# Gaurav14cs17/Bayer_Low_light_Image_Enhancement

Measured on AMD Instinct MI355X. Metric: megapixels/sec RawFormer-S 512x512 RAW->sRGB, higher is better.
Workload: dtype f32; 1 GPU; RawFormer-S(FLCA) dim=32, batch=8 of packed 4x512x512 synthetic Bayer per GPU; frames_per_gpu=8, variant=flca, weights=synthetic (seeded, random-init scale), parallelism=batch-sharded x1, device=AMD Radeon Graphics

## Files before the change

bayer_low_light_image_enhancement_amd/csrc/rf_block.hip:

```cpp
#include <cstdlib>
#include "rf_common.h"

namespace rf {

size_t transformer_scratch_floats(int B, int C, int heads, int hc, int h, int w, TbBufOffsets* o) {
    const size_t P = (size_t)h * w;
    Bump b;
    const size_t wide = (size_t)(3 * C > hc ? 3 * C : hc);
    o->bufA = b.off((size_t)B * wide * P);
    o->bufB = b.off((size_t)B * wide * P);
    o->x1 = b.off((size_t)B * C * P);
    int ns, sl;
    size_t pf = 0, pf2 = 0;
    if (gram_plan(B, C, heads, (int)P, &ns, &sl, &pf)) return 0;
    if (fused_attn_supported(C, heads, h, w)) fused_attn_plan(h, w, &ns, &pf2, B, C);
    if (attn_mid_supported(C, heads, h, w)) attn_mid_plan(h, w, &ns, &pf2, B, C);
    o->partial = b.off(pf > pf2 ? pf : pf2);
    o->wfold = b.off((size_t)B * packed1x1_floats(C, C));
    o->wfold3 = b.off((size_t)B * packed1x1_b3_floats(C, C));
    return b.used;
}

bool transformer_ffn_is_fused(const TbParams& p, int C, int hc, int hh, int ww) {
#ifdef RF_DIAG
// ... 31 lines not shown
            RF_TRY(launch_attn_mid(buf.pre, buf.qkv, partial, nslab, p.qkv_dw_w, p.qkv_dw_b, B, C, hh, ww, st, p.ylo, p.yhi, p.xlo, p.xhi));
            av.x1 = buf.qkv; av.x1_bstride = (int64_t)C * Pn;
        } else {
            DwConvArgs d{};
            d.x = buf.pre; d.x_bstride = (int64_t)3 * C * Pn; d.out = buf.qkv; d.out_bstride = (int64_t)3 * C * Pn;
            d.w = p.qkv_dw_w; d.bias = p.qkv_dw_b;
            d.B = B; d.C = 3 * C; d.h = hh; d.w_ = ww; d.gelu = 0;
            RF_TRY(launch_dwconv3x3(d, st));

            GramArgs g{};
            g.q = buf.qkv; g.k = buf.qkv + (size_t)C * Pn; g.bstride = (int64_t)3 * C * Pn;
            g.B = B; g.C = C; g.heads = heads; g.P = Pn; g.partial = partial;
            RF_TRY(gram_plan(B, C, heads, Pn, &g.nslab, &g.slab, &partial_floats));
            g.p_lo = p.ylo * ww; g.p_hi = p.yhi * ww;
            if (p.xhi > 0 && (p.xlo > 0 || p.xhi < ww)) { g.w = ww; g.x_lo = p.xlo; g.x_hi = p.xhi; }
            RF_TRY(launch_gram(g, st));
            nslab = g.nslab;
            av.x1 = buf.qkv + (size_t)2 * C * Pn; av.x1_bstride = (int64_t)3 * C * Pn;
        }
    }
    if (p.allreduce) p.allreduce(p.allreduce_user, partial, partial_floats, 0, (void*)st);
    RF_TRY(launch_attn_fold(partial, nslab, p.temperature, p.proj_w, buf.wfold, buf.wfold3, B, C, heads, st, p.log_temperature));
    av.C1 = C;
    av.wp = buf.wfold; av.wp_bstride = (int64_t)packed1x1_floats(C, C);
    av.wp3 = buf.wfold3; av.wp3_bstride = (int64_t)packed1x1_b3_floats(C, C);
    av.bias = p.proj_b;
    if (residual) { av.res = in; av.res_bstride = (int64_t)C * Pn; }
    av.out = out; av.out_bstride = (int64_t)C * Pn; av.Cout = C; av.B = B; av.P = Pn; av.w = ww;
    return launch_conv1x1(av, st);
}

int run_transformer(const TbParams& p, const float* in, float* out, float* ws, const TbBufOffsets& o,
                    int B, int C, int heads, int hc, int hh, int ww, hipStream_t st) {
    const int Pn = hh * ww;
    float* bufA = ws + o.bufA;
    float* bufB = ws + o.bufB;
    float* x1 = ws + o.x1;
#ifdef RF_DIAG
    const bool no_fuse = getenv("RF_NO_FUSE") != nullptr;
    const bool no_fuse_attn = no_fuse || getenv("RF_NO_FUSE_ATTN") != nullptr;
#else
    constexpr bool no_fuse = false, no_fuse_attn = false;
#endif

    RF_TRY(run_chan_attn(p, in, x1, true, AttnBufs{bufA, bufB, ws + o.partial, ws + o.wfold, ws + o.wfold3}, B, C, heads, hh, ww, st, no_fuse,
                         no_fuse_attn));

    if (transformer_ffn_is_fused(p, C, hc, hh, ww)) {
        RF_TRY(launch_ffn_fused(x1, out, p.ln2_w, p.ln2_b, p.pw1_wp3, p.pw1_b, p.dw_w, p.dw_b, p.pw2_wp, p.pw2_b, B, C, hh, ww, st));
    } else {
        Conv1x1Args f1{};
        f1.x1 = x1; f1.C1 = C; f1.x1_bstride = (int64_t)C * Pn;
        f1.wp = p.pw1_wp; f1.wp3 = p.pw1_wp3; f1.bias = p.pw1_b;
        f1.ln_w = p.ln2_w; f1.ln_b = p.ln2_b; f1.ln_eps = 1e-5f;
        f1.out = bufA; f1.out_bstride = (int64_t)hc * Pn; f1.Cout = hc; f1.B = B; f1.P = Pn; f1.w = ww;
        if (!conv1x1_ln_single_pass(f1)) {
            RF_TRY(launch_layernorm2d(x1, bufB, p.ln2_w, p.ln2_b, 1e-5f, B, C, Pn, st));
            f1.x1 = bufB; f1.ln_w = nullptr; f1.ln_b = nullptr;
        }
        RF_TRY(launch_conv1x1(f1, st));

        DwConvArgs d2{};
        d2.x = bufA; d2.x_bstride = (int64_t)hc * Pn; d2.out = bufB; d2.out_bstride = (int64_t)hc * Pn;
        d2.w = p.dw_w; d2.bias = p.dw_b;
        d2.B = B; d2.C = hc; d2.h = hh; d2.w_ = ww; d2.gelu = 1;
        RF_TRY(launch_dwconv3x3(d2, st));
        if (p.defer_pw2) return RF_OK;

        Conv1x1Args f2{};
        f2.x1 = bufB; f2.C1 = hc; f2.x1_bstride = (int64_t)hc * Pn;
        f2.wp = p.pw2_wp; f2.wp3 = p.pw2_wp3; f2.bias = p.pw2_b;
        f2.res = x1; f2.res_bstride = (int64_t)C * Pn;
        f2.out = out; f2.out_bstride = (int64_t)C * Pn; f2.Cout = C; f2.B = B; f2.P = Pn; f2.w = ww;
        RF_TRY(launch_conv1x1(f2, st));
    }
    return RF_OK;
}

}
```

bayer_low_light_image_enhancement_amd/csrc/rf_common.h:

```cpp
#pragma once
#include <hip/hip_runtime.h>
#include <stdint.h>
#include <stddef.h>
#include "../../include/rawformer_hip.h"

namespace rf {

typedef float f32x4 __attribute__((ext_vector_type(4)));

void set_error(const char* fmt, ...);
int check_hip(hipError_t e, const char* what);
int check_launch(const char* what);

#define RF_CHECK_ARG(cond, ...)            \
    do {                                   \
        if (!(cond)) {                     \
            rf::set_error(__VA_ARGS__);    \
            return RF_E_INVALID;           \
        }                                  \
    } while (0)

#define RF_TRY(expr)            \
    do {                        \
        const int rc_ = (expr); \
// ... 168 lines not shown
struct DwConvArgs {
    const float* x; int64_t x_bstride;
    float* out; int64_t out_bstride;
    const float* w;
    const float* bias;
    int B, C, h, w_;
    int gelu;
    float* out2 = nullptr;
};
int launch_dwconv3x3(const DwConvArgs& a, hipStream_t st);
int launch_pixel_unshuffle2(const float* in, float* out, int B, int C, int h, int w, hipStream_t st);
int launch_pixel_shuffle2(const float* in, float* out, int B, int C, int h, int w, hipStream_t st);
int launch_dwt2x2(const float* in, float* out, const float k[16], int layout, int exact_haar,
                  int B, int C, int h, int w, int hin, int win, hipStream_t st);
int launch_idwt2x2(const float* in, float* out, const float k[16], int layout, int exact_haar,
                   int B, int C, int h, int w, hipStream_t st);

struct GramArgs {
    const float* q; const float* k;
    int64_t bstride;
    int B, C, heads, P;
    float* partial;
    int nslab, slab;
    int p_lo = 0, p_hi = 0;
    int w = 0, x_lo = 0, x_hi = 0;
};
int gram_plan(int B, int C, int heads, int P, int* nslab, int* slab, size_t* partial_floats);
int launch_gram(const GramArgs& a, hipStream_t st);
int launch_attn_fold(const float* partial, int nslab, const float* temperature, const float* w_out,
                     float* wp_out, void* wp3_out , int B, int C, int heads, hipStream_t st,
                     int log_temperature = 0);

bool fused_ffn_supported(int C, int hidden, int h, int w);
int launch_ffn_fused(const float* x, float* out, const float* ln_w, const float* ln_b, const void* w1p , const float* b1,
                     const float* wd, const float* bd, const float* w2p, const float* b2, int B, int C, int h, int w, hipStream_t st);
bool fused_attn_supported(int C, int heads, int h, int w);
int fused_attn_plan(int h, int w, int* nslab, size_t* partial_floats, int B, int C);
int launch_attn_front(const float* x, float* v, float* partial, int nslab, const float* ln_w, const float* ln_b,
                      const void* wp , const float* bq, const float* wd, const float* bd, int B, int C, int h, int w, hipStream_t st,
                      int ylo = 0, int yhi = 0 ,
                      int xlo = 0, int xhi = 0 );

bool attn_mid_supported(int C, int heads, int h, int w);
int attn_mid_plan(int h, int w, int* nslab, size_t* partial_floats, int B, int C);
int launch_attn_mid(const float* qkv, float* v, float* partial, int nslab, const float* wd, const float* bd,
                    int B, int C, int h, int w, hipStream_t st, int ylo = 0, int yhi = 0, int xlo = 0, int xhi = 0);

struct TbParams {
    const float *ln1_w, *ln1_b, *temperature;
    const float *qkv_wp , *qkv_b, *qkv_dw_w, *qkv_dw_b, *proj_w , *proj_b;
    const float *ln2_w, *ln2_b, *pw1_wp , *pw1_b, *dw_w, *dw_b, *pw2_wp , *pw2_b;
    const void *qkv_wp3, *pw1_wp3, *pw2_wp3;
    int log_temperature;
    int ylo = 0, yhi = 0, xlo = 0, xhi = 0;
    void (*allreduce)(void* user, float* buf, size_t n, int op, void* stream) = nullptr;
    void* allreduce_user = nullptr;
    bool defer_pw2 = false;
};
bool transformer_ffn_is_fused(const TbParams& p, int C, int hc, int hh, int ww);
struct TbBufOffsets { size_t bufA, bufB, x1, partial, wfold, wfold3; };
size_t transformer_scratch_floats(int B, int C, int heads, int hc, int h, int w, TbBufOffsets* o);
int run_transformer(const TbParams& p, const float* in, float* out, float* ws, const TbBufOffsets& o,
                    int B, int C, int heads, int hc, int hh, int ww, hipStream_t st);
struct AttnBufs {
    float *pre, *qkv;
    float *partial;
    float *wfold;
    void* wfold3;
};
int run_chan_attn(const TbParams& p, const float* in, float* out, bool residual, const AttnBufs& buf, int B, int C, int heads, int hh, int ww,
                  hipStream_t st, bool no_fuse = false, bool no_fuse_attn = false);

int launch_rfft2_polar(const float* in, float* mag, float* pha, float2* cscratch, int planes, int h, int w, hipStream_t st);
int launch_polar_irfft2(const float* mag, const float* pha, const float* res, float* out, float2* cscratch, int planes, int h, int w,
                        float lim, hipStream_t st);
int launch_clamp(const float* in, float* out, size_t n, float lo, float hi, hipStream_t st);

size_t tc_front_scratch_floats(int B, int H, int W, int levels);
int launch_tc_front(const float* in, int mosaic, const float* wb_gains, const float* color_matrix, const float* wp_c0, const float* b_c0,
                    const float* wp_c2, const float* b_c2, const float* wp_d0, const float* b_d0, const float* wp_d2, const float* b_d2,
                    float* scratch, int B, int H, int W, int levels, hipStream_t st);
int launch_tc_guide_level(const float* scratch, float* guide, int B, int H, int W, int levels, int hf, int wf, hipStream_t st);
int tc_front_outputs(const float* scratch, const float** y, const float** crcb, const float** rgb, int B, int H, int W, int levels);
int tc_nblk(int h, int w);
int launch_tc_spatial(const float* feat, float* xs, const float* guide, const float* w_col, const float* b_col, const float* w_low,
                      const float* b_low, const float* w_high, const float* b_high, int B, int C, int h, int w, hipStream_t st);
int launch_tc_residual(const float* xs, const float* r, float* x2, float* partial, int B, int C, int h, int w, hipStream_t st);
int launch_tc_color_head(float* x, const float* const* prm, int B, size_t P, hipStream_t st);

size_t gram2_partial_floats(int B, int Ca, int Cb, int h, int w, int ntap);
struct Gram2Launch {
    const float* a; int64_t a_bstride; int Ca;
    const float* b; int64_t b_bstride; int Cb;
    const float* b2; int64_t b2_bstride; int Cb2;
    float* out; int ld;
    size_t out_istride;
// ... 73 lines not shown
```

bayer_low_light_image_enhancement_amd/csrc/rf_fused.hip:

```cpp
#include <cstdio>
#include <cstdlib>
#include "rf_common.h"

namespace rf {

#ifdef RF_STAMP
__device__ unsigned long long g_stamp[16];
#define STAMP_DECL unsigned long long st_prev = __builtin_amdgcn_s_memtime(), st_acc[8] = {0, 0, 0, 0, 0, 0, 0, 0};
#define STAMP(i) do { __builtin_amdgcn_sched_barrier(0); unsigned long long t_ = __builtin_amdgcn_s_memtime(); st_acc[i] += t_ - st_prev; st_prev = t_; __builtin_amdgcn_sched_barrier(0); } while (0)
#define STAMP_FLUSH do { if ((threadIdx.x & 63) == 0) for (int i_ = 0; i_ < 8; ++i_) atomicAdd(&g_stamp[i_], st_acc[i_]); } while (0)
#else
#define STAMP_DECL
#define STAMP(i)
#define STAMP_FLUSH
#endif

__device__ __forceinline__ void lds_barrier() {
    asm volatile("s_waitcnt lgkmcnt(0)" ::: "memory");
    __builtin_amdgcn_s_barrier();
    asm volatile("" ::: "memory");
}

namespace fused {
constexpr int TH = 4, TW = 64;
// ... 171 lines not shown
#pragma unroll
        for (int q = 0; q < 4; ++q) out[q] = fmaf(k2, v[q + 2], fmaf(k1, v[q + 1], fmaf(k0, v[q], out[q])));
    }
}

__device__ __forceinline__ void stencil4_wide(const float* __restrict__ p, const float* __restrict__ k9, float bias, float (&out)[4]) {
    using namespace fused;
#pragma unroll
    for (int q = 0; q < 4; ++q) out[q] = bias;
#pragma unroll
    for (int dy = 0; dy < 3; ++dy) {
        const float* row = p + dy * HC;
        const float4 lft = *reinterpret_cast<const float4*>(row - 4);
        const float4 m = *reinterpret_cast<const float4*>(row);
        const float4 rgt = *reinterpret_cast<const float4*>(row + 4);
        const float v[6] = {lft.w, m.x, m.y, m.z, m.w, rgt.x};
        const float k0 = k9[dy * 3], k1 = k9[dy * 3 + 1], k2 = k9[dy * 3 + 2];
#pragma unroll
        for (int q = 0; q < 4; ++q) out[q] = fmaf(k2, v[q + 2], fmaf(k1, v[q + 1], fmaf(k0, v[q], out[q])));
    }
}

struct FfnArgs {
    const float* x;
    float* out;
    const float* ln_w; const float* ln_b;
    const void* w1p;
    const float* b1;
    const float* wd;
    const float* bd;
    const float* w2p;
    const float* b2;
    int B, h, w, tiles_x, ntiles;
};

template <int C>
__global__ void __launch_bounds__(256, 2) ffn_fused_kernel(FfnArgs a) {
    using namespace fused;
    constexpr int NS = C / 4;
    constexpr int NT1 = 2 * C / 16;
    constexpr int NTO = C / 16;
    constexpr int NPART = 2 * C / PART;
    constexpr int PS = 448;
    __shared__ __attribute__((aligned(16))) float mid[PART * PS + 8];
    __shared__ __attribute__((aligned(16))) u32x4 w1_l[(C / 32) * NT1 * 192];
    __shared__ __attribute__((aligned(16))) float w2_l[(2 * C / 4) * NTO * 64];
    __shared__ float wd_l[2 * C * 9], bd_l[2 * C], b1_l[2 * C], b2_l[C], gam_l[C], bet_l[C];

    const int tid = threadIdx.x, lane = tid & 63, wave = tid >> 6;
    const int j = lane & 15, kq = lane >> 4;
    const int b = blockIdx.y;
    const int h = a.h, w = a.w, P = h * w;
    const float* xb = a.x + (size_t)b * C * P;
    float* ob = a.out + (size_t)b * C * P;

    for (int i = tid; i < (C / 32) * NT1 * 192; i += 256) w1_l[i] = reinterpret_cast<const u32x4*>(a.w1p)[i];
    for (int i = tid; i < (2 * C / 4) * NTO * 16; i += 256) *reinterpret_cast<float4*>(w2_l + i * 4) = *reinterpret_cast<const float4*>(a.w2p + i * 4);
    for (int i = tid; i < 2 * C * 9; i += 256) wd_l[i] = a.wd[i];
    for (int i = tid; i < 2 * C; i += 256) { bd_l[i] = a.bd[i]; b1_l[i] = a.b1[i]; }
    for (int i = tid; i < C; i += 256) { gam_l[i] = a.ln_w[i]; bet_l[i] = a.ln_b[i]; b2_l[i] = a.b2[i]; }
    __syncthreads();
    STAMP_DECL

    const int tiles_y = a.ntiles / a.tiles_x;
    const int per = (a.ntiles + (int)gridDim.x - 1) / (int)gridDim.x;
    const int t_begin = blockIdx.x * per, t_end = (t_begin + per < a.ntiles) ? t_begin + per : a.ntiles;
    for (int tile = t_begin; tile < t_end; ++tile) {
        const int tx = tile / tiles_y, ty = tile % tiles_y;
        const int x0 = tx * TW, y0 = ty * TH;
        STAMP(0);
        const GroupGeom gw0 = group_geom(wave, 0, j, y0, x0, h, w), gw1 = group_geom(wave, 1, j, y0, x0, h, w);
        u32x4 bp0[C / 32][4][3], bp1[C / 32][4][3];
        {
            float4 xh0[NS], xh1[NS];
            load_step_b3<C>(xb, P, kq, gw0, xh0);
            load_step_b3<C>(xb, P, kq, gw1, xh1);
            ln_step_b3<C>(kq, gam_l, bet_l, 1e-5f, xh0);
            ln_step_b3<C>(kq, gam_l, bet_l, 1e-5f, xh1);
            split_step<C>(xh0, bp0);
            split_step<C>(xh1, bp1);
        }
        STAMP(1);

        const int yo = y0 + wave, xo = x0 + 4 * j;
        const bool live = yo < h && xo < w;
        const unsigned voff = (unsigned)(4 * kq) * (unsigned)P + (unsigned)(live ? yo * w + xo : 0);
        float4 resv[NTO * 4];
        f32x4 acc[NTO][4];
#pragma unroll
        for (int t = 0; t < NTO; ++t)
#pragma unroll
            for (int q = 0; q < 4; ++q) acc[t][q] = (f32x4){0.f, 0.f, 0.f, 0.f};

#pragma unroll
        for (int part = 0; part < NPART; ++part) {
            lds_barrier();
            STAMP(0);
            phase_a_step_b3<C, NT1>(bp0, w1_l + lane, 2 * part, 2 * part + 1, b1_l + part * PART, b1_l + part * PART + 16, mid, PS, kq, gw0);
            phase_a_step_b3<C, NT1>(bp1, w1_l + lane, 2 * part, 2 * part + 1, b1_l + part * PART, b1_l + part * PART + 16, mid, PS, kq, gw1);
            STAMP(2);
            if (part == NPART - 1) {
#pragma unroll
                for (int t = 0; t < NTO; ++t)
#pragma unroll
                    for (int r = 0; r < 4; ++r) resv[t * 4 + r] = *reinterpret_cast<const float4*>(xb + (size_t)(16 * t + r) * P + voff);
            }
            lds_barrier();
            STAMP(0);
#pragma unroll
            for (int s = 0; s < PART / 4; ++s) {
                const int hc = 4 * s + kq;
                float v[4];
                stencil4_dpp(mid + hc * PS + wave * HC + 4 * j + 4, j, wd_l + (part * PART + hc) * 9, bd_l[part * PART + hc], v);
#pragma unroll
                for (int q = 0; q < 4; ++q) v[q] = gelu_fast(v[q]);
#pragma unroll
                for (int t = 0; t < NTO; ++t) {
                    const float av = w2_l[((part * (PART / 4) + s) * NTO + t) * 64 + lane];
#pragma unroll
                    for (int q = 0; q < 4; ++q) acc[t][q] = __builtin_amdgcn_mfma_f32_16x16x4f32(av, v[q], acc[t][q], 0, 0, 0);
                }
            }
            STAMP(3);
        }
        if (live) {
#pragma unroll
            for (int t = 0; t < NTO; ++t)
#pragma unroll
                for (int r = 0; r < 4; ++r) {
                    const int cu = 16 * t + r;
                    const float bs = b2_l[cu + 4 * kq];
                    const float4 rv = resv[t * 4 + r];
                    *reinterpret_cast<float4*>(ob + (size_t)cu * P + voff) =
                        make_float4(acc[t][0][r] + bs + rv.x, acc[t][1][r] + bs + rv.y, acc[t][2][r] + bs + rv.z, acc[t][3][r] + bs + rv.w);
                }
        }
        STAMP(4);
    }
    STAMP_FLUSH;
}

namespace fused8 {
constexpr int GPW = 14;
}

__device__ __forceinline__ GroupGeom group_geom8(int wave, int j, int y0, int x0, int h, int w) {
    using namespace fused;
    GroupGeom g;
    const int gi = wave * fused8::GPW + j;
    const bool in_step = j < fused8::GPW && gi < NG;
    const int row = gi / (HC / 4), cg = gi % (HC / 4);
    const int y = y0 - 1 + row, x = x0 - 4 + 4 * cg;
    g.valid = in_step && y >= 0 && y < h && x >= 0 && x < w;
    g.lds_off = in_step ? row * HC + 4 * cg : -1;
    g.goff = g.valid ? y * w + x : 0;
    return g;
}

template <int C, int KP>
__device__ __forceinline__ void load_step_b3p(const float* __restrict__ xb, int P, int kq, const GroupGeom& g, float4 (&xh)[KP / 4]) {
#pragma unroll
    for (int s = 0; s < KP / 4; ++s) {
        const int ch = 32 * (s >> 3) + 8 * kq + (s & 7);
        xh[s] = *reinterpret_cast<const float4*>(xb + (size_t)(ch < C ? ch : 0) * P + (unsigned)g.goff);
    }
}

// ... 130 lines not shown
        }
        lds_barrier();
        if (hf == 0) {
#pragma unroll
            for (int t = 0; t < NTO; ++t)
#pragma unroll
                for (int q = 0; q < 4; ++q) {
                    const float4 o = red[(t * 4 + q) * 256 + row * 64 + lane];
                    acc[t][q][0] += o.x; acc[t][q][1] += o.y; acc[t][q][2] += o.z; acc[t][q][3] += o.w;
                }
            if (live) {
#pragma unroll
                for (int t = 0; t < NTO; ++t)
#pragma unroll
                    for (int r = 0; r < 4; ++r) {
                        const int cu = 16 * t + r;
                        const float bs = b2_l[cu + 4 * kq];
                        const float4 rv = resv[t * 4 + r];
                        *reinterpret_cast<float4*>(ob + (size_t)cu * P + voff) =
                            make_float4(acc[t][0][r] + bs + rv.x, acc[t][1][r] + bs + rv.y, acc[t][2][r] + bs + rv.z, acc[t][3][r] + bs + rv.w);
                    }
            }
        }
    }
}

bool fused_ffn_supported(int C, int hidden, int h, int w) {
#ifdef RF_DIAG
    if (C == 64 && getenv("RF_FFN8_64") && hidden == 2 * C && (w % 4 == 0) && ((double)C * h * w * 4.0 < 4.0e9)) return true;
#endif
    return (C == 32 || C == 48) && hidden == 2 * C && (w % 4 == 0) && ((double)C * h * w * 4.0 < 4.0e9);
}

int launch_ffn_fused(const float* x, float* out, const float* ln_w, const float* ln_b, const void* w1p, const float* b1,
                     const float* wd, const float* bd, const float* w2p, const float* b2, int B, int C, int h, int w, hipStream_t st) {
    RF_CHECK_ARG((C == 32 || C == 48 || C == 64) && w % 4 == 0 && (double)C * h * w * 4.0 < 4.0e9 && B <= 65535, "ffn_fused: unsupported shape C=%d %dx%d", C, h, w);
    RF_CHECK_ARG(aligned16(x) && aligned16(out) && aligned16(w1p), "ffn_fused: buffers must be 16-byte aligned");
    FfnArgs a{x, out, ln_w, ln_b, w1p, b1, wd, bd, w2p, b2, B, h, w, cdiv(w, fused::TW), 0};
    a.ntiles = a.tiles_x * cdiv(h, fused::TH);
    int wgs = cdiv(512, B);
    if (wgs > a.ntiles) wgs = a.ntiles;
    const dim3 grid((unsigned)wgs, (unsigned)B);
    const double px = (double)B * h * w;
    if (C != 32) {
        int wg8 = cdiv(256, B);
        if (wg8 > a.ntiles) wg8 = a.ntiles;
        const dim3 grid8((unsigned)wg8, (unsigned)B);
        ProfScope prof(st, C == 64 ? "ffn_fused8_kernel<64>" : "ffn_fused8_kernel<48>", px * (8.0 * C * C + 36.0 * C), px * 8.0 * C);
        if (C == 64) ffn_fused8_kernel<64><<<grid8, 512, 0, st>>>(a);
        else ffn_fused8_kernel<48><<<grid8, 512, 0, st>>>(a);
        return check_launch("ffn_fused8");
    }
    ProfScope prof(st, "ffn_fused_kernel<32>", px * (8.0 * C * C + 36.0 * C), px * 8.0 * C);
    ffn_fused_kernel<32><<<grid, 256, 0, st>>>(a);
    return check_launch("ffn_fused");
}

struct AttnFrontArgs {
    const float* x;
    float* v;
    float* partial;
    const float* ln_w; const float* ln_b;
    const void* wp;
    const float* bq;
    const float* wd;
    const float* bd;
    int B, h, w, tiles_x, ntiles, nslab;
    int ylo, yhi;
    int xlo, xhi;
};

template <int C>
__global__ void __launch_bounds__(256, 2) attn_front_kernel(AttnFrontArgs a) {
    using namespace fused;
    constexpr int NS = C / 4;
    constexpr int NQT = C / 16;
    constexpr int NVP = C / PART;
    constexpr int NT3 = 3 * C / 16;
    constexpr int PSG = fused::PSG;
    constexpr int PSV = 448;
    constexpr int ROWW = 4 * 16 + 2;
    __shared__ __attribute__((aligned(16))) float mid[PART * PSG + 8];
    __shared__ __attribute__((aligned(16))) u32x4 w_l[(C / 32) * NT3 * 192];
    __shared__ float wd_l[3 * C * 9], bd_l[3 * C], bq_l[3 * C], gam_l[C], bet_l[C];

    const int tid = threadIdx.x, lane = tid & 63, wave = tid >> 6;
    const int j = lane & 15, kq = lane >> 4;
// ... 360 lines not shown
```

bayer_low_light_image_enhancement_amd/csrc/rf_model.hip:

```cpp
#include <string>
#include <unordered_map>
#include <vector>
#include <cstring>
#include <cstdlib>
#include "rf_common.h"

using namespace rf;

#include "rf_handle.h"

namespace {

int add_param(rf_handle* h, const std::string& name, std::initializer_list<int64_t> shape) {
    Param p;
    p.name = name;
    p.ndim = (int)shape.size();
    int i = 0;
    for (auto s : shape) p.shape[i++] = s;
    for (; i < 4; ++i) p.shape[i] = 1;
    p.ptr = nullptr;
    h->index[name] = (int)h->params.size();
    h->params.push_back(p);
    return (int)h->params.size() - 1;
}
// ... 180 lines not shown
    const rf_config& cfg = h->cfg;
    const StageIx& x = h->stage[i];
    const int lvl = x.lvl, C = cfg.dim << lvl, hh = H >> lvl, ww = W >> lvl, Pn = hh * ww, heads = cfg.heads[lvl];
    const int hc = C * cfg.ffn_expansion;
    float* trans = ws + p.trans;
    float* xs = ws + p.xs;
    float* crb = ws + p.cr;

    TbParams tp{};
    tp.ln1_w = h->prm(x.ln1_w); tp.ln1_b = h->prm(x.ln1_b);
    tp.temperature = h->prm(x.temperature); tp.log_temperature = cfg.variant == RF_VARIANT_TRUECOLOR;
    tp.qkv_wp = h->pk(x.qkv_w); tp.qkv_b = h->prm(x.qkv_b);
    tp.qkv_dw_w = h->prm(x.qkv_dw_w); tp.qkv_dw_b = h->prm(x.qkv_dw_b);
    tp.proj_w = h->prm(x.proj_w); tp.proj_b = h->prm(x.proj_b);
    tp.ln2_w = h->prm(x.ln2_w); tp.ln2_b = h->prm(x.ln2_b);
    tp.pw1_wp = h->pk(x.pw1_w); tp.pw1_b = h->prm(x.pw1_b);
    tp.dw_w = h->prm(x.dw_w); tp.dw_b = h->prm(x.dw_b);
    tp.pw2_wp = h->pk(x.pw2_w); tp.pw2_b = h->prm(x.pw2_b);
    tp.qkv_wp3 = h->pk3(x.qkv_w); tp.pw1_wp3 = h->pk3(x.pw1_w); tp.pw2_wp3 = h->pk3(x.pw2_w);
    const bool sharded = h->shard_allreduce != nullptr;
    const int ylo = sharded ? h->shard_y_lo >> lvl : 0, yhi = sharded ? h->shard_y_hi >> lvl : 0;
    const int xlo = sharded ? h->shard_x_lo >> lvl : 0, xhi = sharded ? h->shard_x_hi >> lvl : 0;
    const int P_pool = sharded ? (h->shard_total_rows >> lvl) * (h->shard_total_cols ? h->shard_total_cols >> lvl : ww) : Pn;
    if (sharded) {
        tp.ylo = ylo; tp.yhi = yhi; tp.xlo = xlo; tp.xhi = xhi;
        tp.allreduce = h->shard_allreduce; tp.allreduce_user = h->shard_user;
    }
    TbBufOffsets to{p.bufA, p.bufB, p.x1, p.gram_partial, p.wfold_attn, p.wfold_attn3};
    bool compose = x.tail_offset != 0 && Pn % 4 == 0 && !transformer_ffn_is_fused(tp, C, hc, hh, ww);
#ifdef RF_DIAG
    if (getenv("RF_NO_COMPOSE") || getenv("RF_NO_B3")) compose = false;
#endif
    tp.defer_pw2 = compose;
    const float* composed = compose ? h->packed + x.tail_offset : nullptr;
    if (cfg.variant == RF_VARIANT_TRUECOLOR) RF_TRY(run_transformer(tp, in, trans, ws, to, B, C, heads, hc, hh, ww, st));
    else RF_TRY(h->side.fork(st, side));

    Conv1x1Args r{};
    r.x1 = xs; r.C1 = C; r.x1_bstride = (int64_t)C * Pn;
    r.x2 = trans; r.C2 = C; r.x2_bstride = (int64_t)C * Pn;
    r.bias = h->prm(x.cr_b);
    r.out = crb; r.out_bstride = (int64_t)C * Pn; r.Cout = C; r.B = B; r.P = Pn; r.w = ww;
    if (cfg.variant == RF_VARIANT_TRUECOLOR) {
        const TcIx& t = x.tc;
        RF_TRY(launch_tc_spatial(in, xs, ws + p.guide[lvl], h->prm(t.col_w), h->prm(t.col_b), h->prm(t.low_w), h->prm(t.low_b), h->prm(t.high_w),
                                 h->prm(t.high_b), B, C, hh, ww, st));
        Conv1x1Args r0{};
        r0.x1 = xs; r0.C1 = C; r0.x1_bstride = (int64_t)C * Pn; r0.wp = h->pk(t.res0_w); r0.wp3 = h->pk3(t.res0_w);
        r0.bias = h->prm(t.res0_b); r0.out = crb; r0.out_bstride = (int64_t)C * Pn; r0.Cout = C; r0.B = B; r0.P = Pn; r0.w = ww; r0.act = 2;
        RF_TRY(launch_conv1x1(r0, st));
        Conv1x1Args r2 = r0;
        r2.x1 = crb; r2.wp = h->pk(t.res2_w); r2.wp3 = h->pk3(t.res2_w); r2.bias = h->prm(t.res2_b);
        r2.out = ws + p.bufA; r2.act = 0;
        RF_TRY(launch_conv1x1(r2, st));
        RF_TRY(launch_tc_residual(xs, ws + p.bufA, xs, ws + p.flca_partial, B, C, hh, ww, st));
        RF_TRY(launch_flca_se_fold(ws + p.flca_partial, tc_nblk(hh, ww), Pn, h->se_prm(t.se), h->prm(x.cr_w), ws + p.wfold_cr, ws + p.wfold_cr3,
                                   ws + p.ch, B, C, st, composed, hc));
        r.wp = ws + p.wfold_cr; r.wp_bstride = (int64_t)packed1x1_floats(2 * C, C);
        r.wp3 = ws + p.wfold_cr3; r.wp3_bstride = (int64_t)packed1x1_b3_floats(compose ? 2 * C + hc : 2 * C, C);
    } else if (cfg.variant == RF_VARIANT_FLCA) {
        const FlcaPrm fp = h->flca_prm(x.flca);
        FlcaSpatialArgs s{};
        s.feat = in; s.xs = xs; s.guide = ws + p.guide[lvl];
        s.set_params(fp);
        s.partial = ws + p.flca_partial; s.B = B; s.C = C; s.h = hh; s.w = ww; s.nblk = flca_nblk(hh, ww);
        s.ylo = ylo; s.yhi = yhi; s.xlo = xlo; s.xhi = xhi;
        RF_TRY(launch_flca_spatial(s, side));
        if (sharded) h->shard_allreduce(h->shard_user, s.partial, (size_t)B * s.nblk * C, 0, (void*)side);
        RF_TRY(launch_flca_se_fold(s.partial, s.nblk, P_pool, fp.se, h->prm(x.cr_w), ws + p.wfold_cr, ws + p.wfold_cr3, ws + p.ch, B, C, side,
                                   composed, hc));
        r.wp = ws + p.wfold_cr; r.wp_bstride = (int64_t)packed1x1_floats(2 * C, C);
        r.wp3 = ws + p.wfold_cr3; r.wp3_bstride = (int64_t)packed1x1_b3_floats(compose ? 2 * C + hc : 2 * C, C);
    } else {
        Conv3x3Args cb{};
        cb.x = in; cb.x_bstride = (int64_t)C * Pn; cb.wp = h->pk(x.conv_w); cb.bias = h->prm(x.conv_b);
        cb.out = xs; cb.out_bstride = (int64_t)C * Pn; cb.B = B; cb.Cin = C; cb.Cout = C; cb.h = hh; cb.w = ww;
        cb.act = cfg.branch_lrelu ? 1 : 0;
        RF_TRY(launch_conv3x3(cb, side));
        r.wp = h->pk(x.cr_w);
        r.wp3 = compose ? h->packed + x.tail3_offset : h->pk3(x.cr_w);
    }
    if (cfg.variant != RF_VARIANT_TRUECOLOR) {
        RF_TRY(run_transformer(tp, in, trans, ws, to, B, C, heads, hc, hh, ww, st));
        RF_TRY(h->side.join(st, side));
    }
    if (compose) {
        r.wp = nullptr;
        r.x2 = ws + p.x1;
        r.x3 = ws + p.bufB; r.C3 = hc; r.x3_bstride = (int64_t)hc * Pn;
        r.bias = composed + (size_t)C * hc;
    }
    RF_TRY(launch_conv1x1(r, st));

    Conv3x3Args co{};
    co.x = crb; co.x_bstride = (int64_t)C * Pn; co.wp = h->pk(x.out_w); co.bias = h->prm(x.out_b);
    co.out = out; co.out_bstride = (int64_t)C * Pn; co.B = B; co.Cin = C; co.Cout = C; co.h = hh; co.w = ww; co.act = 1;
    if (p.ks_floats) { co.ks_scratch = ws + p.ks; co.ks_floats = p.ks_floats; }
    RF_TRY(launch_conv3x3(co, st));
    return RF_OK;
}

}

hipStream_t SideStream::get(hipStream_t st) {
    if (failed || profiling_active()) return st;
    if (!stream &&
        (hipStreamCreateWithFlags(&stream, hipStreamNonBlocking) != hipSuccess ||
         hipEventCreateWithFlags(&ev_fork, hipEventDisableTiming) != hipSuccess ||
         hipEventCreateWithFlags(&ev_join, hipEventDisableTiming) != hipSuccess)) {
        (void)hipGetLastError();
        destroy();
        failed = true;
        return st;
    }
    return stream;
}

int SideStream::fork(hipStream_t st, hipStream_t side) {
    if (side == st) return RF_OK;
    pending = true;
    ++forks;
    RF_TRY(check_hip(hipEventRecord(ev_fork, st), "side stream fork (record)"));
    RF_TRY(check_hip(hipStreamWaitEvent(side, ev_fork, 0), "side stream fork (wait)"));
#ifdef RF_DIAG
    const char* n = getenv("RF_FAIL_FORK");
// ... 373 lines not shown
```

bayer_low_light_image_enhancement_amd/isa_check.py:

```python
from __future__ import annotations

import os
import re
import shutil
import subprocess
import tempfile

LLVM_BIN = "/opt/rocm/lib/llvm/bin"
_PK_F32 = re.compile(r"^\s*(v_pk_(?:fma|mul|add)_f32)\s+(.*)$")
_MOD = re.compile(r"\b(op_sel|op_sel_hi|neg_lo|neg_hi):\[([01,]+)\]")


def _split_operands(rest: str):
    m = _MOD.search(rest)
    ops, mods = (rest[:m.start()], rest[m.start():]) if m else (rest, "")
    comment = ""
    for mark in ("//", ";"):
        if mark in ops:
            ops, comment = ops.split(mark, 1)[0], mark + ops.split(mark, 1)[1]
    return [o.strip() for o in ops.strip().rstrip(",").split(",") if o.strip()], mods, comment


def is_vulnerable(line: str) -> bool:
    m = _PK_F32.match(line)
# ... 27 lines not shown
    for ln in asm_text.split("\n"):
        if is_vulnerable(ln):
            new = commute_line(ln)
            assert not is_vulnerable(new), (ln, new)
            out.append(new)
            n += 1
        else:
            out.append(ln)
    return "\n".join(out), n


def _tool(name: str) -> str:
    exe = os.path.join(LLVM_BIN, name)
    if not os.path.exists(exe):
        found = shutil.which(name)
        if not found:
            raise RuntimeError(f"{name} not found (needed to inspect the gfx950 code objects)")
        exe = found
    return exe


def extract_code_objects(path: str, outdir: str):
    local = os.path.join(outdir, os.path.basename(path))
    shutil.copy(path, local)
    subprocess.run([_tool("llvm-objdump"), "--offloading", os.path.basename(local)], cwd=outdir, check=True, capture_output=True)
    return sorted(os.path.join(outdir, f) for f in os.listdir(outdir) if "amdgcn-amd-amdhsa--gfx950" in f)


def scan_library(path: str):
    report = {}
    with tempfile.TemporaryDirectory(prefix="rf_isa_") as tmp:
        for co in extract_code_objects(path, tmp):
            notes = subprocess.run([_tool("llvm-readelf"), "--notes", co], check=True, capture_output=True, text=True).stdout
            cur = None
            for ln in notes.splitlines():
                t = ln.strip()
                if t.startswith(".name:"):
                    cur = t.split(":", 1)[1].strip()
                    report.setdefault(cur, {"scratch": 0, "vgpr_spill": 0, "sgpr_spill": 0, "vgprs": 0, "vulnerable": []})
                elif cur and t.startswith(".private_segment_fixed_size:"):
                    report[cur]["scratch"] = int(t.split(":")[1])
                elif cur and t.startswith(".vgpr_spill_count:"):
                    report[cur]["vgpr_spill"] = int(t.split(":")[1])
                elif cur and t.startswith(".sgpr_spill_count:"):
                    report[cur]["sgpr_spill"] = int(t.split(":")[1])
                elif cur and t.startswith(".vgpr_count:"):
                    report[cur]["vgprs"] = int(t.split(":")[1])
            dis = subprocess.run([_tool("llvm-objdump"), "-d", co], check=True, capture_output=True, text=True).stdout
            cur = None
            for ln in dis.splitlines():
                m = re.match(r"^[0-9a-f]+ <(\S+)>:", ln)
                if m:
                    cur = m.group(1)
                    continue
                if cur and is_vulnerable(ln):
                    report.setdefault(cur, {"scratch": 0, "vgpr_spill": 0, "sgpr_spill": 0, "vgprs": 0, "vulnerable": []})
                    report[cur]["vulnerable"].append(ln.split("//")[0].strip())
    return report
```

Baseline: 1074 MP/s.

## Fuse stage-tail channel-reduce 1x1 conv into fused FFN kernel epilogue

Adds a TAIL variant of the fused FFN kernel. It computes the stage's channel-reduce 1x1 conv over the concatenated side-branch and transformer outputs in the epilogue, using the composed FFN-out weights plus the per-batch folded weights via extra MFMAs. This removes the separate conv1x1 launch and the write and re-read of the transformer output. In exchange, the side stream must join before the FFN instead of after, which reduces overlap. The kernel also takes on more register pressure and per-lane global weight loads.

After: 1096 MP/s (median of 6 runs). +2.0%, better.

```diff
diff --git a/bayer_low_light_image_enhancement_amd/csrc/rf_block.hip b/bayer_low_light_image_enhancement_amd/csrc/rf_block.hip
--- a/bayer_low_light_image_enhancement_amd/csrc/rf_block.hip
+++ b/bayer_low_light_image_enhancement_amd/csrc/rf_block.hip
@@ -87,7 +87,12 @@
 
 int run_transformer(const TbParams& p, const float* in, float* out, float* ws, const TbBufOffsets& o,
                     int B, int C, int heads, int hc, int hh, int ww, hipStream_t st) {
-    const int Pn = hh * ww;
+    RF_TRY(run_transformer_attn(p, in, ws, o, B, C, heads, hh, ww, st));
+    return run_transformer_ffn(p, out, ws, o, B, C, hc, hh, ww, st);
+}
+
+int run_transformer_attn(const TbParams& p, const float* in, float* ws, const TbBufOffsets& o, int B, int C, int heads, int hh, int ww,
+                         hipStream_t st) {
     float* bufA = ws + o.bufA;
     float* bufB = ws + o.bufB;
     float* x1 = ws + o.x1;
@@ -98,12 +103,19 @@
     constexpr bool no_fuse = false, no_fuse_attn = false;
 #endif
 
-    RF_TRY(run_chan_attn(p, in, x1, true, AttnBufs{bufA, bufB, ws + o.partial, ws + o.wfold, ws + o.wfold3}, B, C, heads, hh, ww, st, no_fuse,
-                         no_fuse_attn));
+    return run_chan_attn(p, in, x1, true, AttnBufs{bufA, bufB, ws + o.partial, ws + o.wfold, ws + o.wfold3}, B, C, heads, hh, ww, st, no_fuse,
+                         no_fuse_attn);
+}
 
+int run_transformer_ffn(const TbParams& p, float* out, float* ws, const TbBufOffsets& o, int B, int C, int hc, int hh, int ww, hipStream_t st) {
+    const int Pn = hh * ww;
+    float* bufA = ws + o.bufA;
+    float* bufB = ws + o.bufB;
+    float* x1 = ws + o.x1;
     if (transformer_ffn_is_fused(p, C, hc, hh, ww)) {
-        RF_TRY(launch_ffn_fused(x1, out, p.ln2_w, p.ln2_b, p.pw1_wp3, p.pw1_b, p.dw_w, p.dw_b, p.pw2_wp, p.pw2_b, B, C, hh, ww, st));
+        RF_TRY(launch_ffn_fused(x1, out, p.ln2_w, p.ln2_b, p.pw1_wp3, p.pw1_b, p.dw_w, p.dw_b, p.pw2_wp, p.pw2_b, B, C, hh, ww, st, p.tail));
     } else {
+        RF_CHECK_ARG(!p.tail.xs, "run_transformer: the stage tail needs the fused FFN kernel");
         Conv1x1Args f1{};
         f1.x1 = x1; f1.C1 = C; f1.x1_bstride = (int64_t)C * Pn;
         f1.wp = p.pw1_wp; f1.wp3 = p.pw1_wp3; f1.bias = p.pw1_b;
diff --git a/bayer_low_light_image_enhancement_amd/csrc/rf_common.h b/bayer_low_light_image_enhancement_amd/csrc/rf_common.h
--- a/bayer_low_light_image_enhancement_amd/csrc/rf_common.h
+++ b/bayer_low_light_image_enhancement_amd/csrc/rf_common.h
@@ -224,8 +224,18 @@
                      int log_temperature = 0);
 
 bool fused_ffn_supported(int C, int hidden, int h, int w);
+struct FfnTail {
+    const float* xs = nullptr;
+    const float* w = nullptr;
+    int64_t w_bstride = 0;
+    const float* wc = nullptr;
+    const float* bias = nullptr;
+};
+bool fused_ffn_tail_supported(int C, int hidden, int h, int w);
+bool fused_ffn_tail_fills_grid(int B, int h, int w);
 int launch_ffn_fused(const float* x, float* out, const float* ln_w, const float* ln_b, const void* w1p , const float* b1,
-                     const float* wd, const float* bd, const float* w2p, const float* b2, int B, int C, int h, int w, hipStream_t st);
+                     const float* wd, const float* bd, const float* w2p, const float* b2, int B, int C, int h, int w, hipStream_t st,
+                     const FfnTail& tail = FfnTail());
 bool fused_attn_supported(int C, int heads, int h, int w);
 int fused_attn_plan(int h, int w, int* nslab, size_t* partial_floats, int B, int C);
 int launch_attn_front(const float* x, float* v, float* partial, int nslab, const float* ln_w, const float* ln_b,
@@ -248,12 +258,15 @@
     void (*allreduce)(void* user, float* buf, size_t n, int op, void* stream) = nullptr;
     void* allreduce_user = nullptr;
     bool defer_pw2 = false;
+    FfnTail tail;
 };
 bool transformer_ffn_is_fused(const TbParams& p, int C, int hc, int hh, int ww);
 struct TbBufOffsets { size_t bufA, bufB, x1, partial, wfold, wfold3; };
 size_t transformer_scratch_floats(int B, int C, int heads, int hc, int h, int w, TbBufOffsets* o);
 int run_transformer(const TbParams& p, const float* in, float* out, float* ws, const TbBufOffsets& o,
                     int B, int C, int heads, int hc, int hh, int ww, hipStream_t st);
+int run_transformer_attn(const TbParams& p, const float* in, float* ws, const TbBufOffsets& o, int B, int C, int heads, int hh, int ww, hipStream_t st);
+int run_transformer_ffn(const TbParams& p, float* out, float* ws, const TbBufOffsets& o, int B, int C, int hc, int hh, int ww, hipStream_t st);
 struct AttnBufs {
     float *pre, *qkv;
     float *partial;
diff --git a/bayer_low_light_image_enhancement_amd/csrc/rf_fused.hip b/bayer_low_light_image_enhancement_amd/csrc/rf_fused.hip
--- a/bayer_low_light_image_enhancement_amd/csrc/rf_fused.hip
+++ b/bayer_low_light_image_enhancement_amd/csrc/rf_fused.hip
@@ -227,9 +227,13 @@
     const float* w2p;
     const float* b2;
     int B, h, w, tiles_x, ntiles;
+    const float* xs;
+    const float* wt;
+    int64_t wt_bstride;
+    const float* wc;
 };
 
-template <int C>
+template <int C, bool TAIL>
 __global__ void __launch_bounds__(256, 2) ffn_fused_kernel(FfnArgs a) {
     using namespace fused;
     constexpr int NS = C / 4;
@@ -248,9 +252,19 @@
     const int h = a.h, w = a.w, P = h * w;
     const float* xb = a.x + (size_t)b * C * P;
     float* ob = a.out + (size_t)b * C * P;
+    constexpr int NKT = 2 * C / 4;
+    const float* xsb = TAIL ? a.xs + (size_t)b * C * P : nullptr;
+    const float* wtb = TAIL ? a.wt + (size_t)b * a.wt_bstride : nullptr;
 
     for (int i = tid; i < (C / 32) * NT1 * 192; i += 256) w1_l[i] = reinterpret_cast<const u32x4*>(a.w1p)[i];
-    for (int i = tid; i < (2 * C / 4) * NTO * 16; i += 256) *reinterpret_cast<float4*>(w2_l + i * 4) = *reinterpret_cast<const float4*>(a.w2p + i * 4);
+    if constexpr (TAIL) {
+        for (int i = tid; i < (2 * C / 4) * NTO * 64; i += 256) {
+            const int l = i & 63, t = (i >> 6) % NTO, s = (i >> 6) / NTO;
+            w2_l[i] = a.wc[(16 * t + (l & 15)) * (2 * C) + 4 * s + (l >> 4)];
+        }
+    } else {
+        for (int i = tid; i < (2 * C / 4) * NTO * 16; i += 256) *reinterpret_cast<float4*>(w2_l + i * 4) = *reinterpret_cast<const float4*>(a.w2p + i * 4);
+    }
     for (int i = tid; i < 2 * C * 9; i += 256) wd_l[i] = a.wd[i];
     for (int i = tid; i < 2 * C; i += 256) { bd_l[i] = a.bd[i]; b1_l[i] = a.b1[i]; }
     for (int i = tid; i < C; i += 256) { gam_l[i] = a.ln_w[i]; bet_l[i] = a.ln_b[i]; b2_l[i] = a.b2[i]; }
@@ -280,7 +294,9 @@
         const int yo = y0 + wave, xo = x0 + 4 * j;
         const bool live = yo < h && xo < w;
         const unsigned voff = (unsigned)(4 * kq) * (unsigned)P + (unsigned)(live ? yo * w + xo : 0);
-        float4 resv[NTO * 4];
+        float4 resv[TAIL ? 1 : NTO * 4];
+        float4 tb[TAIL ? NKT : 1];
+        float ta[TAIL ? NKT * NTO : 1];
         f32x4 acc[NTO][4];
 #pragma unroll
         for (int t = 0; t < NTO; ++t)
@@ -295,10 +311,23 @@
             phase_a_step_b3<C, NT1>(bp1, w1_l + lane, 2 * part, 2 * part + 1, b1_l + part * PART, b1_l + part * PART + 16, mid, PS, kq, gw1);
             STAMP(2);
             if (part == NPART - 1) {
-#pragma unroll
-                for (int t = 0; t < NTO; ++t)
-#pragma unroll
-                    for (int r = 0; r < 4; ++r) resv[t * 4 + r] = *reinterpret_cast<const float4*>(xb + (size_t)(16 * t + r) * P + voff);
+                if constexpr (TAIL) {
+                    const unsigned toff = (unsigned)kq * (unsigned)P + (unsigned)(live ? yo * w + xo : 0);
+                    int lane_t = lane;
+                    asm volatile("" : "+v"(lane_t));
+#pragma unroll
+                    for (int s = 0; s < C / 4; ++s) {
+                        tb[s] = *reinterpret_cast<const float4*>(xsb + (size_t)(4 * s) * P + toff);
+                        tb[C / 4 + s] = *reinterpret_cast<const float4*>(xb + (size_t)(4 * s) * P + toff);
+                    }
+#pragma unroll
+                    for (int i = 0; i < NKT * NTO; ++i) ta[i] = wtb[i * 64 + lane_t];
+                } else {
+#pragma unroll
+                    for (int t = 0; t < NTO; ++t)
+#pragma unroll
+                        for (int r = 0; r < 4; ++r) resv[t * 4 + r] = *reinterpret_cast<const float4*>(xb + (size_t)(16 * t + r) * P + voff);
+                }
             }
             lds_barrier();
             STAMP(0);
@@ -318,6 +347,16 @@
             }
             STAMP(3);
         }
+        if constexpr (TAIL) {
+#pragma unroll
+            for (int s = 0; s < NKT; ++s) {
+                const float bv[4] = {tb[s].x, tb[s].y, tb[s].z, tb[s].w};
+#pragma unroll
+                for (int t = 0; t < NTO; ++t)
+#pragma unroll
+                    for (int q = 0; q < 4; ++q) acc[t][q] = __builtin_amdgcn_mfma_f32_16x16x4f32(ta[s * NTO + t], bv[q], acc[t][q], 0, 0, 0);
+            }
+        }
         if (live) {
 #pragma unroll
             for (int t = 0; t < NTO; ++t)
@@ -325,9 +364,13 @@
                 for (int r = 0; r < 4; ++r) {
                     const int cu = 16 * t + r;
                     const float bs = b2_l[cu + 4 * kq];
-                    const float4 rv = resv[t * 4 + r];
-                    *reinterpret_cast<float4*>(ob + (size_t)cu * P + voff) =
-                        make_float4(acc[t][0][r] + bs + rv.x, acc[t][1][r] + bs + rv.y, acc[t][2][r] + bs + rv.z, acc[t][3][r] + bs + rv.w);
+                    float4* dst = reinterpret_cast<float4*>(ob + (size_t)cu * P + voff);
+                    if constexpr (TAIL) {
+                        *dst = make_float4(acc[t][0][r] + bs, acc[t][1][r] + bs, acc[t][2][r] + bs, acc[t][3][r] + bs);
+                    } else {
+                        const float4 rv = resv[t * 4 + r];
+                        *dst = make_float4(acc[t][0][r] + bs + rv.x, acc[t][1][r] + bs + rv.y, acc[t][2][r] + bs + rv.z, acc[t][3][r] + bs + rv.w);
+                    }
                 }
         }
         STAMP(4);
@@ -524,13 +567,20 @@
     return (C == 32 || C == 48) && hidden == 2 * C && (w % 4 == 0) && ((double)C * h * w * 4.0 < 4.0e9);
 }
 
+bool fused_ffn_tail_supported(int C, int hidden, int h, int w) { return C == 32 && fused_ffn_supported(C, hidden, h, w); }
+constexpr int kFfnGrid = 512;
+bool fused_ffn_tail_fills_grid(int B, int h, int w) { return (long)B * cdiv(w, fused::TW) * cdiv(h, fused::TH) >= kFfnGrid; }
+
 int launch_ffn_fused(const float* x, float* out, const float* ln_w, const float* ln_b, const void* w1p, const float* b1,
-                     const float* wd, const float* bd, const float* w2p, const float* b2, int B, int C, int h, int w, hipStream_t st) {
+                     const float* wd, const float* bd, const float* w2p, const float* b2, int B, int C, int h, int w, hipStream_t st,
+                     const FfnTail& tail) {
     RF_CHECK_ARG((C == 32 || C == 48 || C == 64) && w % 4 == 0 && (double)C * h * w * 4.0 < 4.0e9 && B <= 65535, "ffn_fused: unsupported shape C=%d %dx%d", C, h, w);
     RF_CHECK_ARG(aligned16(x) && aligned16(out) && aligned16(w1p), "ffn_fused: buffers must be 16-byte aligned");
-    FfnArgs a{x, out, ln_w, ln_b, w1p, b1, wd, bd, w2p, b2, B, h, w, cdiv(w, fused::TW), 0};
+    RF_CHECK_ARG(!tail.xs || (C == 32 && tail.w && tail.wc && tail.bias && aligned16(tail.xs)),
+                 "ffn_fused: the stage tail needs C = 32 and 16-byte aligned operands (C = %d)", C);
+    FfnArgs a{x, out, ln_w, ln_b, w1p, b1, wd, bd, w2p, tail.xs ? tail.bias : b2, B, h, w, cdiv(w, fused::TW), 0, tail.xs, tail.w, tail.w_bstride, tail.wc};
     a.ntiles = a.tiles_x * cdiv(h, fused::TH);
-    int wgs = cdiv(512, B);
+    int wgs = cdiv(kFfnGrid, B);
     if (wgs > a.ntiles) wgs = a.ntiles;
     const dim3 grid((unsigned)wgs, (unsigned)B);
     const double px = (double)B * h * w;
@@ -543,8 +593,13 @@
         else ffn_fused8_kernel<48><<<grid8, 512, 0, st>>>(a);
         return check_launch("ffn_fused8");
     }
-    ProfScope prof(st, "ffn_fused_kernel<32>", px * (8.0 * C * C + 36.0 * C), px * 8.0 * C);
-    ffn_fused_kernel<32><<<grid, 256, 0, st>>>(a);
+    if (tail.xs) {
+        ProfScope prof(st, "ffn_fused_kernel<32, true>", px * (12.0 * C * C + 36.0 * C), px * 12.0 * C);
+        ffn_fused_kernel<32, true><<<grid, 256, 0, st>>>(a);
+        return check_launch("ffn_fused_tail");
+    }
+    ProfScope prof(st, "ffn_fused_kernel<32, false>", px * (8.0 * C * C + 36.0 * C), px * 8.0 * C);
+    ffn_fused_kernel<32, false><<<grid, 256, 0, st>>>(a);
     return check_launch("ffn_fused");
 }
 
diff --git a/bayer_low_light_image_enhancement_amd/csrc/rf_model.hip b/bayer_low_light_image_enhancement_amd/csrc/rf_model.hip
--- a/bayer_low_light_image_enhancement_amd/csrc/rf_model.hip
+++ b/bayer_low_light_image_enhancement_amd/csrc/rf_model.hip
@@ -236,7 +236,22 @@
     if (getenv("RF_NO_COMPOSE") || getenv("RF_NO_B3")) compose = false;
 #endif
     tp.defer_pw2 = compose;
-    const float* composed = compose ? h->packed + x.tail_offset : nullptr;
+    bool fuse_tail = x.tail_offset != 0 && cfg.variant != RF_VARIANT_TRUECOLOR && transformer_ffn_is_fused(tp, C, hc, hh, ww) &&
+                     fused_ffn_tail_supported(C, hc, hh, ww);
+    bool tail_any_size = false;
+#ifdef RF_DIAG
+    if (getenv("RF_NO_FUSE_TAIL")) fuse_tail = false;
+    tail_any_size = getenv("RF_FUSE_TAIL_ANY_SIZE") != nullptr;
+#endif
+    if (!tail_any_size && !fused_ffn_tail_fills_grid(B, hh, ww)) fuse_tail = false;
+    const float* composed = (compose || fuse_tail) ? h->packed + x.tail_offset : nullptr;
+    if (fuse_tail) {
+        tp.tail.xs = xs;
+        tp.tail.wc = composed;
+        tp.tail.bias = composed + (size_t)C * hc;
+        if (cfg.variant == RF_VARIANT_FLCA) { tp.tail.w = ws + p.wfold_cr; tp.tail.w_bstride = (int64_t)packed1x1_floats(2 * C, C); }
+        else tp.tail.w = h->pk(x.cr_w);
+    }
     if (cfg.variant == RF_VARIANT_TRUECOLOR) RF_TRY(run_transformer(tp, in, trans, ws, to, B, C, heads, hc, hh, ww, st));
     else RF_TRY(h->side.fork(st, side));
 
@@ -271,22 +286,28 @@
         s.ylo = ylo; s.yhi = yhi; s.xlo = xlo; s.xhi = xhi;
         RF_TRY(launch_flca_spatial(s, side));
         if (sharded) h->shard_allreduce(h->shard_user, s.partial, (size_t)B * s.nblk * C, 0, (void*)side);
-        RF_TRY(launch_flca_se_fold(s.partial, s.nblk, P_pool, fp.se, h->prm(x.cr_w), ws + p.wfold_cr, ws + p.wfold_cr3, ws + p.ch, B, C, side,
-                                   composed, hc));
-        r.wp = ws + p.wfold_cr; r.wp_bstride = (int64_t)packed1x1_floats(2 * C, C);
-        r.wp3 = ws + p.wfold_cr3; r.wp3_bstride = (int64_t)packed1x1_b3_floats(compose ? 2 * C + hc : 2 * C, C);
+        RF_TRY(launch_flca_se_fold(s.partial, s.nblk, P_pool, fp.se, h->prm(x.cr_w), ws + p.wfold_cr, fuse_tail ? nullptr : ws + p.wfold_cr3,
+                                   ws + p.ch, B, C, side, compose ? composed : nullptr, hc));
+        if (!fuse_tail) {
+            r.wp = ws + p.wfold_cr; r.wp_bstride = (int64_t)packed1x1_floats(2 * C, C);
+            r.wp3 = ws + p.wfold_cr3; r.wp3_bstride = (int64_t)packed1x1_b3_floats(compose ? 2 * C + hc : 2 * C, C);
+        }
     } else {
         Conv3x3Args cb{};
         cb.x = in; cb.x_bstride = (int64_t)C * Pn; cb.wp = h->pk(x.conv_w); cb.bias = h->prm(x.conv_b);
         cb.out = xs; cb.out_bstride = (int64_t)C * Pn; cb.B = B; cb.Cin = C; cb.Cout = C; cb.h = hh; cb.w = ww;
         cb.act = cfg.branch_lrelu ? 1 : 0;
         RF_TRY(launch_conv3x3(cb, side));
-        r.wp = h->pk(x.cr_w);
-        r.wp3 = compose ? h->packed + x.tail3_offset : h->pk3(x.cr_w);
+        if (!fuse_tail) {
+            r.wp = h->pk(x.cr_w);
+            r.wp3 = compose ? h->packed + x.tail3_offset : h->pk3(x.cr_w);
+        }
     }
     if (cfg.variant != RF_VARIANT_TRUECOLOR) {
-        RF_TRY(run_transformer(tp, in, trans, ws, to, B, C, heads, hc, hh, ww, st));
-        RF_TRY(h->side.join(st, side));
+        RF_TRY(run_transformer_attn(tp, in, ws, to, B, C, heads, hh, ww, st));
+        if (fuse_tail) RF_TRY(h->side.join(st, side));
+        RF_TRY(run_transformer_ffn(tp, fuse_tail ? crb : trans, ws, to, B, C, hc, hh, ww, st));
+        if (!fuse_tail) RF_TRY(h->side.join(st, side));
     }
     if (compose) {
         r.wp = nullptr;
@@ -294,7 +315,7 @@
         r.x3 = ws + p.bufB; r.C3 = hc; r.x3_bstride = (int64_t)hc * Pn;
         r.bias = composed + (size_t)C * hc;
     }
-    RF_TRY(launch_conv1x1(r, st));
+    if (!fuse_tail) RF_TRY(launch_conv1x1(r, st));
 
     Conv3x3Args co{};
     co.x = crb; co.x_bstride = (int64_t)C * Pn; co.wp = h->pk(x.out_w); co.bias = h->prm(x.out_b);
diff --git a/bayer_low_light_image_enhancement_amd/isa_check.py b/bayer_low_light_image_enhancement_amd/isa_check.py
--- a/bayer_low_light_image_enhancement_amd/isa_check.py
+++ b/bayer_low_light_image_enhancement_amd/isa_check.py
@@ -83,12 +83,17 @@
     with tempfile.TemporaryDirectory(prefix="rf_isa_") as tmp:
         for co in extract_code_objects(path, tmp):
             notes = subprocess.run([_tool("llvm-readelf"), "--notes", co], check=True, capture_output=True, text=True).stdout
-            cur = None
+            cur = lds = None
             for ln in notes.splitlines():
                 t = ln.strip()
-                if t.startswith(".name:"):
+                if t.startswith(".group_segment_fixed_size:"):
+                    lds = int(t.split(":")[1])
+                elif t.startswith(".name:"):
                     cur = t.split(":", 1)[1].strip()
                     report.setdefault(cur, {"scratch": 0, "vgpr_spill": 0, "sgpr_spill": 0, "vgprs": 0, "vulnerable": []})
+                    if lds is not None:
+                        report[cur]["lds"] = lds
+                        lds = None
                 elif cur and t.startswith(".private_segment_fixed_size:"):
                     report[cur]["scratch"] = int(t.split(":")[1])
                 elif cur and t.startswith(".vgpr_spill_count:"):
```
